# microsoft/aurora

Hardware: AMD Instinct MI355X
Metric: forecast-steps/sec (6h step) 0.25deg ERA5 721x1440x13 (higher is better)
Workload: dtype bf16; 1 GPU; AuroraPretrained(autocast=True) 1.3B, 0.25deg ERA5 721x1440, 13 levels, T=2, batch 1 per GPU, one forward step (BASELINE.json configs[1]); parallelism=1 GPU

## Files before the change

aurora_amd/csrc/model.h:

```cpp
#pragma once

#include <math.h>
#include <stdlib.h>
#include <string.h>

#include <algorithm>
#include <array>
#include <exception>
#include <map>
#include <memory>
#include <stdexcept>
#include <string>
#include <vector>

#include "band.h"
#include "common.h"

namespace aurora {

struct Fail {
  int code;
};
#define REQUIRE(cond, ...)               \
  do {                                   \
// ... 175 lines not shown
  std::vector<std::array<int, 2>> merge_pad;

  aurora_hip_band band{0, 1, nullptr, nullptr, nullptr};
  std::vector<std::vector<std::array<int, 2>>> rows;
  std::map<std::pair<int, int>, aurora::DevPlan> plans;
  void* stage_send = nullptr;
  void* stage_recv = nullptr;
  int64_t staging_bytes = 0, staging_need = 0;
  bool sharded() const { return band.world > 1; }
  int fuse_ln = 1;
  bool split_attention = false;
  bool qkv_planes = true;
  bool reassoc_out = true;
  bool compose_front = true;
  bool front_composed = false;
  bool score_weights = true;

  aurora::DevBuf abs_enc, dyn_planes, ctx_max;
  float guard_limit_min[4] = {INFINITY, INFINITY, INFINITY, INFINITY};
  int guard_launches[4] = {0, 0, 0, 0};
  void note_guard(const float* word, float limit) {
    const ptrdiff_t i = word - ctx_max.f();
    if (dry || word == nullptr || i < 0 || i >= 4) return;
    guard_limit_min[i] = std::min(guard_limit_min[i], limit);
    ++guard_launches[i];
  }
  aurora::DevBuf tickets;
  bool split_k = true;
  int abs_B = 0;
  struct Pinned { float* host = nullptr; size_t bytes = 0; hipEvent_t done = nullptr; };
// ... 125 lines not shown
    else linear(op.f32_mode(mode));
  }
  void linear_planes(const void* A, int64_t lda, const void* Wt, int64_t ldw, const float* bias, void* C, int64_t plane_stride,
                     int heads, int64_t M, int N, int K) {
    timed(m, stream, K_LINEAR_BF16, 2.0 * (double)M * N * K, [&] {
      return aurora_hip_linear_planes(A, lda, Wt, ldw, bias, C, plane_stride, heads, M, N, K, AURORA_BF16, stream);
    });
  }
  void layernorm(const void* y, int64_t ldy, const float* gain, const float* shift, const float* res, int64_t ldr,
                 int64_t res_mod, float* out_f32, int64_t ldo, void* out_t, int64_t ldt, int64_t M, int D, float eps,
                 int dtype) {
    timed(m, stream, K_LAYERNORM, 0.0, [&] {
      return aurora_hip_layernorm(y, ldy, gain, shift, res, ldr, res_mod, out_f32, ldo, out_t, ldt, M, D, eps, dtype, stream);
    });
  }
  void layernorm_split(const float* y, int64_t ldy, const float* gain, const float* shift, const void* res, int64_t ldr,
                       int64_t res_mod, int res_is_split, float* out_f32, int64_t ldo, void* out_split, int64_t ld_split,
                       int64_t M, int D, float eps) {
    timed(m, stream, K_LAYERNORM, 0.0, [&] {
      return aurora_hip_layernorm_split(y, ldy, gain, shift, res, ldr, res_mod, res_is_split, out_f32, ldo, out_split, ld_split, M, D,
                                        eps, stream);
    });
  }
  void perceiver_attention(const PerceiverCols& g, int head_dim, const float* q, int64_t q_stride, const float* kv, float* att,
                           const float* pair_word, float pair_limit, const float* skip_word, float skip_limit) {
    timed(m, stream, K_PERCEIVER_ATTENTION, 0.0, [&] {
      if (skip_word)
        return aurora_hip_perceiver_attention_unless(q, q_stride, kv, att, g.B, g.cols, g.kv_bstride, g.kv_lstride, g.Lq, g.Lk, g.heads,
                                                     head_dim, AURORA_F32, pair_word, pair_limit, skip_word, skip_limit, stream);
      return aurora_hip_perceiver_attention_ex(q, q_stride, kv, att, g.B, g.cols, g.kv_bstride, g.kv_lstride, g.Lq, g.Lk, g.heads,
// ... 81 lines not shown
```

aurora_amd/csrc/model.hip:

```cpp
#include "model.h"

namespace aurora {

hipEvent_t take_event(Model& m) {
  if (!m.event_pool.empty()) {
    hipEvent_t e = m.event_pool.back();
    m.event_pool.pop_back();
    return e;
  }
  hipEvent_t e;
  hip_ok(hipEventCreate(&e), "hipEventCreate");
  return e;
}

int bounded_mode() {
  static const int mode = getenv("AURORA_F32_GEMM") ? -1 : 2;
  return mode;
}

std::string level_to_str(double level) {
  const double value = round(level * 1000.0) / 1000.0;
  char buf[64];
  if (value == (double)(long long)value) snprintf(buf, sizeof buf, "%lld", (long long)value);
  else {
// ... 162 lines not shown
    build_channels(*m);
    m->ctx_max = DevBuf(16);
    const auto& tu = c->tuning;
    REQUIRE(tu.fuse_ln >= 0 && tu.fuse_ln <= 3, "create: tuning.fuse_ln = %d (0 default, 1 never, 2 by the fill rule, 3 always)", tu.fuse_ln);
    auto sw = [](int32_t v, bool dflt, const char* what) {
      REQUIRE(v >= 0 && v <= 2, "create: tuning.%s = %d (0 default, 1 off, 2 on)", what, v);
      return v == 0 ? dflt : v == 2;
    };
    m->fuse_ln = tu.fuse_ln == 0 ? 1 : tu.fuse_ln - 1;
    m->split_attention = sw(tu.band_split_attention, false, "band_split_attention");
    m->qkv_planes = sw(tu.qkv_planes, true, "qkv_planes");
    m->split_k = sw(tu.split_k, true, "split_k");
    m->reassoc_out = sw(tu.perceiver_reassoc, true, "perceiver_reassoc");
    m->score_weights = sw(tu.score_weights, true, "score_weights");
    m->compose_front = sw(tu.compose_front, true, "compose_front");
    m->tickets = DevBuf(SPLIT_TICKETS * sizeof(int32_t));
    hip_ok(hipMemset(m->tickets.p, 0, SPLIT_TICKETS * sizeof(int32_t)), "hipMemset");
    *out = m.release();
  })
}

extern "C" void aurora_hip_destroy(aurora_hip_model* m) { delete m; }

extern "C" int aurora_hip_set_band(aurora_hip_model* mp, const aurora_hip_band* band) {
  GUARDED({
    REQUIRE(mp != nullptr, "set_band: null model");
    Model& m = *mp;
    if (band == nullptr || band->world <= 1) {
      m.band = aurora_hip_band{0, 1, nullptr, nullptr, nullptr};
    } else {
// ... 168 lines not shown
```

aurora_amd/csrc/norm.hip:

```cpp
#include <stdlib.h>

#include "common.h"

namespace aurora {
namespace {

constexpr int ROWS_PER_BLOCK = 4;

template <int MAXC>
__device__ __forceinline__ void row_stats(const float (&v)[MAXC][8], int lane, int n_pieces, float inv_d, float eps,
                                          float& mean, float& rstd) {
  float s = 0.f;
#pragma unroll
  for (int i = 0; i < MAXC; ++i)
    if (lane + 64 * i < n_pieces) {
#pragma unroll
      for (int j = 0; j < 8; ++j) s += v[i][j];
    }
  mean = wave_sum(s) * inv_d;
  float q = 0.f;
#pragma unroll
  for (int i = 0; i < MAXC; ++i)
    if (lane + 64 * i < n_pieces) {
#pragma unroll
      for (int j = 0; j < 8; ++j) {
        const float d = v[i][j] - mean;
        q = fmaf(d, d, q);
      }
    }
  rstd = rsqrtf(wave_sum(q) * inv_d + eps);
}

struct LnArgs {
  const void* y; int64_t ldy; const float* gain; const float* shift;
  const float* res; int64_t ldr; int64_t res_mod;
  float* out_f32; int64_t ldo; void* out_t; int64_t ldt;
  int64_t M; int D; float eps;
  int split_t;
  int split_res;
};

template <typename T, int NC, bool PRE = false>
__global__ __launch_bounds__(256) void layernorm_f32_kernel(const LnArgs p) {
  const int lane = threadIdx.x & 63;
  const int64_t row = (int64_t)blockIdx.x * ROWS_PER_BLOCK + (threadIdx.x >> 6);
  if (row >= p.M) return;
  const int n_pieces = p.D >> 2;
  const T* yr = reinterpret_cast<const T*>(p.y) + row * p.ldy;
  const float* rr = nullptr;
  if (p.res) rr = p.res + (p.res_mod > 0 ? (int64_t)(((p.M | p.res_mod) >> 32) == 0 ? (uint32_t)row % (uint32_t)p.res_mod : row % p.res_mod) : row) * p.ldr;
  const bool res_plain = PRE && rr != nullptr && !p.split_res;
  float v[NC][4], r4[PRE ? NC : 1][4];
#pragma unroll
  for (int i = 0; i < NC; ++i)
    if (lane + 64 * i < n_pieces) {
      load4(yr + (lane + 64 * i) * 4, v[i]);
      if constexpr (PRE) {
        if (res_plain) load4(rr + (lane + 64 * i) * 4, r4[i]);
      }
    }
  float s = 0.f;
#pragma unroll
  for (int i = 0; i < NC; ++i)
    if (lane + 64 * i < n_pieces) s += (v[i][0] + v[i][1]) + (v[i][2] + v[i][3]);
  const float inv_d = 1.0f / p.D;
  const float mean = wave_sum(s) * inv_d;
  float q = 0.f;
#pragma unroll
  for (int i = 0; i < NC; ++i)
    if (lane + 64 * i < n_pieces) {
#pragma unroll
      for (int j = 0; j < 4; ++j) {
        const float d = v[i][j] - mean;
        q = fmaf(d, d, q);
      }
    }
  const float rstd = rsqrtf(wave_sum(q) * inv_d + p.eps);
#pragma unroll
  for (int i = 0; i < NC; ++i) {
    const int e = (lane + 64 * i) * 4;
    if (lane + 64 * i < n_pieces) {
      float gn[4], sh[4], o[4];
      if (p.gain) load4(p.gain + e, gn);
      if (p.shift) load4(p.shift + e, sh);
#pragma unroll
      for (int j = 0; j < 4; ++j) {
        float t = (v[i][j] - mean) * rstd;
        if (p.gain) t *= gn[j];
        if (p.shift) t += sh[j];
        o[j] = t;
      }
      if (rr && p.split_res) {
        const char* s = reinterpret_cast<const char*>(rr) + (e & ~31) * 4 + (e & 31) * 2;
        const u32x2 h = *reinterpret_cast<const u32x2*>(s);
        const u32x2 l = *reinterpret_cast<const u32x2*>(s + 64);
        auto half = [](uint32_t w, int hi) { return (float)__builtin_bit_cast(_Float16, (uint16_t)(hi ? w >> 16 : w & 0xffffu)); };
        const uint32_t hw[2] = {h.x, h.y}, lw[2] = {l.x, l.y};
#pragma unroll
        for (int j = 0; j < 4; ++j) o[j] += half(hw[j >> 1], j & 1) + half(lw[j >> 1], j & 1);
      } else if (rr) {
        if constexpr (PRE) {
#pragma unroll
          for (int j = 0; j < 4; ++j) o[j] += r4[i][j];
        } else {
          float r[4];
          load4(rr + e, r);
#pragma unroll
          for (int j = 0; j < 4; ++j) o[j] += r[j];
        }
      }
      if (p.out_f32) store4(p.out_f32 + row * p.ldo + e, o);
      if (p.out_t && p.split_t) {
        uint32_t h0, h1, l0, l1;
        split_pair_f16(o[0], o[1], h0, l0);
        split_pair_f16(o[2], o[3], h1, l1);
        const bool odd = (lane & 1) != 0;
        auto swap1 = [](uint32_t x) { return (uint32_t)__builtin_amdgcn_update_dpp(0, (int)x, 0xB1, 0xf, 0xf, true); };
        const uint32_t r0 = swap1(odd ? h0 : l0), r1 = swap1(odd ? h1 : l1);
        const int e8 = e & ~7;
        char* d = reinterpret_cast<char*>(p.out_t) + (row * p.ldt + (e8 & ~31)) * 4 + (e8 & 31) * 2 + (odd ? 64 : 0);
        *reinterpret_cast<u32x4*>(d) = odd ? u32x4{r0, r1, l0, l1} : u32x4{h0, h1, r0, r1};
      } else if (p.out_t) {
        store4(reinterpret_cast<T*>(p.out_t) + row * p.ldt + e, o);
      }
    }
  }
}

struct MergeArgs {
  const float* x; const float* w; const float* b; void* out;
  int B, C, H, W, D, H2, W2; float eps;
};

template <typename T, int MAXC>
__global__ __launch_bounds__(256) void merge_ln_kernel(const MergeArgs p) {
  const int lane = threadIdx.x & 63;
  const int64_t row = (int64_t)blockIdx.x * ROWS_PER_BLOCK + (threadIdx.x >> 6);
  const int64_t rows = (int64_t)p.B * p.C * p.H2 * p.W2;
  if (row >= rows) return;
// ... 77 lines not shown
}
}

using namespace aurora;

#define AURORA_DISPATCH_ROW(KERNEL, T, D, ...)                                                        \
  do {                                                                                                \
    if ((D) <= 512) hipLaunchKernelGGL((KERNEL<T, 1>), __VA_ARGS__);                                  \
    else if ((D) <= 1024) hipLaunchKernelGGL((KERNEL<T, 2>), __VA_ARGS__);                            \
    else if ((D) <= 2048) hipLaunchKernelGGL((KERNEL<T, 4>), __VA_ARGS__);                            \
    else hipLaunchKernelGGL((KERNEL<T, 8>), __VA_ARGS__);                                             \
  } while (0)

static int layernorm_impl(const void* y, int64_t ldy, const float* gain, const float* shift, const float* res, int64_t ldr,
                          int64_t res_mod, float* out_f32, int64_t ldo, void* out_t, int64_t ldt, int64_t M, int D,
                          float eps, int dtype, int split_t, int split_res, void* stream);

extern "C" int aurora_hip_layernorm(const void* y, int64_t ldy, const float* gain, const float* shift,
                                    const float* res, int64_t ldr, int64_t res_mod, float* out_f32,
                                    int64_t ldo, void* out_t, int64_t ldt, int64_t M, int D, float eps,
                                    int dtype, void* stream) {
  return layernorm_impl(y, ldy, gain, shift, res, ldr, res_mod, out_f32, ldo, out_t, ldt, M, D, eps, dtype, 0, 0, stream);
}

extern "C" int aurora_hip_layernorm_split(const float* y, int64_t ldy, const float* gain, const float* shift,
                                          const void* res, int64_t ldr, int64_t res_mod, int res_is_split, float* out_f32,
                                          int64_t ldo, void* out_split, int64_t ld_split, int64_t M, int D, float eps,
                                          void* stream) {
  AURORA_CHECK_ARG(D % 32 == 0, "layernorm_split: D=%d must be a multiple of 32", D);
  AURORA_CHECK_ARG(out_split == nullptr || (ld_split % 32 == 0 && ld_split >= D),
                   "layernorm_split: the pair-layout output stride must be a multiple of 32, >= D");
  AURORA_CHECK_ARG(!res_is_split || (res != nullptr && ldr % 32 == 0 && ldr >= D),
                   "layernorm_split: the pair-layout residual stride must be a multiple of 32, >= D");
  return layernorm_impl(y, ldy, gain, shift, static_cast<const float*>(res), ldr, res_mod, out_f32, ldo, out_split, ld_split,
                        M, D, eps, AURORA_F32, out_split ? 1 : 0, res_is_split ? 1 : 0, stream);
}

static int layernorm_impl(const void* y, int64_t ldy, const float* gain, const float* shift, const float* res, int64_t ldr,
                          int64_t res_mod, float* out_f32, int64_t ldo, void* out_t, int64_t ldt, int64_t M, int D,
                          float eps, int dtype, int split_t, int split_res, void* stream) {
  AURORA_CHECK_ARG(dtype == AURORA_F32 || dtype == AURORA_BF16, "layernorm: bad dtype");
  AURORA_CHECK_ARG(D % 8 == 0 && D > 0 && D <= 4096, "layernorm: D=%d must be a multiple of 8, <= 4096", D);
  const int es = dtype == AURORA_F32 ? 4 : 2;
  AURORA_CHECK_ARG((ldy * es) % 16 == 0 && (uintptr_t)y % 16 == 0, "layernorm: unaligned input rows");
  AURORA_CHECK_ARG((!res || ((ldr * 4) % 16 == 0 && (uintptr_t)res % 16 == 0)) &&
                       (!out_f32 || ((ldo * 4) % 16 == 0 && (uintptr_t)out_f32 % 16 == 0)) &&
                       (!out_t || ((ldt * es) % 16 == 0 && (uintptr_t)out_t % 16 == 0)),
                   "layernorm: unaligned residual/output rows");
  AURORA_CHECK_ARG(out_f32 || out_t, "layernorm: no output");
  if (M <= 0) return AURORA_OK;
  LnArgs p{y, ldy, gain, shift, res, ldr, res_mod, out_f32, ldo, out_t, ldt, M, D, eps, split_t, split_res};
  if (dtype == AURORA_F32) {
    const dim3 grid(row_blocks(M)), block(256);
    if (D <= 256) hipLaunchKernelGGL((layernorm_f32_kernel<float, 1>), grid, block, 0, as_stream(stream), p);
    else if (D <= 512) hipLaunchKernelGGL((layernorm_f32_kernel<float, 2>), grid, block, 0, as_stream(stream), p);
    else if (D <= 1024) hipLaunchKernelGGL((layernorm_f32_kernel<float, 4>), grid, block, 0, as_stream(stream), p);
    else if (D <= 2048) hipLaunchKernelGGL((layernorm_f32_kernel<float, 8>), grid, block, 0, as_stream(stream), p);
    else hipLaunchKernelGGL((layernorm_f32_kernel<float, 16>), grid, block, 0, as_stream(stream), p);
  } else {
    const dim3 grid(row_blocks(M)), block(256);
    const bool pre = res != nullptr && M <= (int64_t)40 * device_cus();
    if (pre) {
      if (D <= 256) hipLaunchKernelGGL((layernorm_f32_kernel<bf16_t, 1, true>), grid, block, 0, as_stream(stream), p);
      else if (D <= 512) hipLaunchKernelGGL((layernorm_f32_kernel<bf16_t, 2, true>), grid, block, 0, as_stream(stream), p);
      else if (D <= 1024) hipLaunchKernelGGL((layernorm_f32_kernel<bf16_t, 4, true>), grid, block, 0, as_stream(stream), p);
      else if (D <= 2048) hipLaunchKernelGGL((layernorm_f32_kernel<bf16_t, 8, true>), grid, block, 0, as_stream(stream), p);
// ... 41 lines not shown
```

aurora_amd/csrc/step.hip:

```cpp
#include <algorithm>

#include "model.h"
#include "resampler_space.h"

namespace aurora {

namespace {

struct CtxGuard { float* word; float a, c, limit_kv; bool pairs, scan; };
struct ComposedFront { const ComposedCtx* layers; int levels, groups; int64_t rows; float embed_l1, embed_bias_max; };

struct ResamplerCall {
  const Resampler* rs;
  const float* ctx;
  int64_t ctx_rows;
  int ctx_dim;
  const float *q0, *latents0;
  PerceiverCols g;
  float eps;
  bool out_pairs;
  const ComposedFront* front;
  CtxGuard guard;
};

// ... 445 lines not shown
    window_attention(s, blk, qkv, plane_stride, ao, (const int32_t*)pl.tok.p, pl.has_grp ? (const uint8_t*)pl.grp.p : nullptr,
                     pl.n_windows, pl.n_tok, Lq, Ls);
  return ao;
}

void block(Step& s, const Block& blk, const void* w_qkv, const void* w_proj, int stage, float* xf, void* xb, float* final_out,
           int64_t final_ld) {
  Model& m = s.m;
  Launcher& L = s.L;
  Arena& A = m.arena;
  const Res res = s.local_res(stage);
  const int64_t Ls = (int64_t)res.c * res.h * res.w, M = (int64_t)s.B * Ls;
  const int dim = blk.dim, bb = s.bb;
  const size_t es = s.es;
  const void* a_in = s.bf ? xb : (const void*)xf;
  const size_t mark = A.top;
  void* ao = s.sharded ? attention_band(s, blk, w_qkv, stage, a_in, Ls) : attention_whole(s, blk, w_qkv, stage, a_in, Ls);
  const int fuse_env = m.fuse_ln;
  const int64_t ln_tiles = (M + 127) / 128, cus = device_cus();
  const bool fills = (double)ln_tiles >= 0.85 * (double)(((ln_tiles + cus - 1) / cus) * cus);
  const bool fuse = s.bf && dim == 512 && (fuse_env == 2 || (fuse_env == 1 && fills));
  auto fused = [&](const void* a, const void* w, const float* bias, int K_, const float* gain, const float* shift, float* xo,
                   int64_t ldo, void* xbo) {
    timed(m, L.stream, K_LINEAR_LN, 2.0 * (double)M * dim * K_, [&] {
      return aurora_hip_linear_layernorm(a, K_, w, K_, bias, gain, shift, xf, dim, xo, ldo, xbo, dim, M, dim, K_, 1e-5f, L.stream);
    });
  };
  if (fuse) {
    fused(ao, w_proj, blk.proj_b, dim, blk.gain1, blk.shift1, xf, dim, xb);
  } else {
    void* y = A.take((size_t)M * dim * es);
    L.linear(LinearOp(ao, dim, w_proj, dim, blk.proj_b, y, dim, M, dim, dim, bb));
    L.layernorm(y, dim, blk.gain1, blk.shift1, xf, dim, 0, xf, dim, xb, dim, M, dim, 1e-5f, bb);
  }
  A.top = mark;
  void* hid = A.take((size_t)M * blk.hidden * es);
  L.linear(LinearOp(a_in, dim, blk.fc1_w, dim, blk.fc1_b, hid, blk.hidden, M, blk.hidden, dim, bb).activation(AURORA_ACT_GELU));
  float* xo = final_out ? final_out : xf;
  const int64_t ldo = final_out ? final_ld : dim;
  void* xbo = final_out ? nullptr : xb;
  if (fuse) {
    fused(hid, blk.fc2_w, blk.fc2_b, blk.hidden, blk.gain2, blk.shift2, xo, ldo, xbo);
  } else {
    void* y2 = A.take((size_t)M * dim * es);
    L.linear(LinearOp(hid, blk.hidden, blk.fc2_w, blk.hidden, blk.fc2_b, y2, dim, M, dim, blk.hidden, bb));
    L.layernorm(y2, dim, blk.gain2, blk.shift2, xf, dim, 0, xo, ldo, xbo, dim, M, dim, 1e-5f, bb);
  }
  A.top = mark;
}

void merge_stage(Step& s, int i, float*& xf, void*& xb) {
  Model& m = s.m;
  Arena& A = m.arena;
  const Res g = m.stage_res[i], r = s.local_res(i);
  REQUIRE(g.h > 1 && g.w > 1, "grid (%d, %d, %d) too small to merge", g.c, g.h, g.w);
  const int dim = m.stage_dim(i);
  const int H2 = (r.h + 1) / 2, W2 = (r.w + 1) / 2;
  REQUIRE(H2 == s.local_res(i + 1).h, "band rows of stages %d / %d do not nest", i, i + 1);
  const int64_t M2 = (int64_t)s.B * r.c * H2 * W2;
  float* nf = (float*)A.take((size_t)M2 * 2 * dim * 4);
  void* nb = s.bf ? A.take((size_t)M2 * 2 * dim * 2) : nullptr;
// ... 248 lines not shown
```

aurora_amd/engine/lib.py:

```python

from __future__ import annotations

import ctypes
import os
import threading
from collections import namedtuple
from ctypes import c_float, c_int, c_int32, c_int64, c_void_p
from pathlib import Path
from typing import Optional

import numpy as np
import torch

from aurora_amd.engine.tables import DeviceTables, _upload

F32, BF16, F64 = 0, 1, 2
ACT_NONE, ACT_GELU, ACT_SILU = 0, 1, 2

_LIB_PATH = Path(__file__).resolve().parents[1] / "_lib" / "libaurora_hip.so"


class PatchVar(ctypes.Structure):
    _fields_ = [
        ("src", c_void_p), ("stride_b", c_int64), ("stride_t", c_int64), ("stride_c", c_int64),
# ... 31 lines not shown
    "aurora_hip_linear_batched": (c_int, [c_void_p, c_int64, c_void_p, c_int64, c_void_p, c_void_p, c_int64, c_int64, c_int,
                                          c_int, c_int, c_int, c_int, c_void_p, c_float, c_int, c_int64, c_int64, c_int64,
                                          c_int64, c_void_p]),
    "aurora_hip_linear_plan": (c_int, [c_int64, c_int, c_int, c_int, c_int, c_int, c_int, c_int64, c_int64, c_int64, c_int64,
                                       c_int64, c_int64, c_int64, c_int, c_int, c_int64, c_int, c_int,
                                       ctypes.POINTER(c_int32)]),
    "aurora_hip_absmax": (c_int, [c_void_p, c_int64, c_void_p, c_void_p]),
    "aurora_hip_absmax_fold": (c_int, [c_void_p, c_int64, c_void_p, c_void_p]),
    "aurora_hip_zero_words": (c_int, [c_void_p, c_int, c_void_p]),
    "aurora_hip_linear_layernorm": (c_int, [c_void_p, c_int64, c_void_p, c_int64, c_void_p, c_void_p, c_void_p, c_void_p,
                                            c_int64, c_void_p, c_int64, c_void_p, c_int64, c_int64, c_int, c_int, c_float,
                                            c_void_p]),
    "aurora_hip_split_f16": (c_int, [c_void_p, c_int64, c_void_p, c_int64, c_int64, c_int, c_float, c_void_p]),
    "aurora_hip_layernorm_split": (c_int, [c_void_p, c_int64, c_void_p, c_void_p, c_void_p, c_int64, c_int64, c_int,
                                           c_void_p, c_int64, c_void_p, c_int64, c_int64, c_int, c_float, c_void_p]),
    "aurora_hip_linear": (c_int, [c_void_p, c_int64, c_void_p, c_int64, c_void_p, c_void_p, c_int64,
                                  c_void_p, c_int64, c_void_p, c_int64, c_int64, c_int, c_int, c_int,
                                  c_int, c_void_p]),
    "aurora_hip_window_attention": (c_int, [c_void_p, c_void_p, c_void_p, c_void_p, c_void_p, c_int,
                                            c_int64, c_int64, c_int, c_int, c_int, c_int, c_int, c_void_p]),
    "aurora_hip_window_attention_planes": (c_int, [c_void_p, c_int64, c_void_p, c_void_p, c_void_p, c_void_p, c_int,
                                                   c_int64, c_int64, c_int, c_int, c_int, c_int, c_int, c_void_p]),
    "aurora_hip_linear_planes": (c_int, [c_void_p, c_int64, c_void_p, c_int64, c_void_p, c_void_p, c_int64, c_int, c_int64,
                                         c_int, c_int, c_int, c_void_p]),
    "aurora_hip_gather_rows": (c_int, [c_void_p, c_int64, c_void_p, c_void_p, c_int64, c_int64, c_int64,
                                       c_void_p]),
    "aurora_hip_layernorm": (c_int, [c_void_p, c_int64, c_void_p, c_void_p, c_void_p, c_int64, c_int64,
                                     c_void_p, c_int64, c_void_p, c_int64, c_int64, c_int, c_float,
                                     c_int, c_void_p]),
    "aurora_hip_merge_ln": (c_int, [c_void_p, c_void_p, c_void_p, c_void_p, c_int, c_int, c_int, c_int,
# ... 429 lines not shown
    nbytes = M * D * (y.element_size() + (4 if res is not None else 0) + (4 if out_f32 is not None else 0)
                      + (y.element_size() if out_t is not None else 0))
    if split_t or split_res:
        assert y.dtype == torch.float32 and (out_t is not None) == split_t and (res is not None or not split_res)
        with _Timed("layernorm", float(nbytes)):
            _check(load().aurora_hip_layernorm_split(_ptr(y), ldy, _ptr(gain), _ptr(shift), _ptr(res), ldr, res_mod,
                                                     1 if split_res else 0, _ptr(out_f32), ldo, _ptr(out_t), ldt, M, D,
                                                     eps, _stream()))
        return
    with _Timed("layernorm", float(nbytes)):
        _check(load().aurora_hip_layernorm(_ptr(y), ldy, _ptr(gain), _ptr(shift), _ptr(res), ldr, res_mod,
                                           _ptr(out_f32), ldo, _ptr(out_t), ldt, M, D, eps,
                                           dtype_code(y.dtype), _stream()))


def merge_ln(x: torch.Tensor, ln_w: torch.Tensor, ln_b: torch.Tensor, out: torch.Tensor,
             B: int, C: int, H: int, W: int, D: int, eps: float = 1e-5) -> torch.Tensor:
    assert x.dtype == torch.float32 and x.is_contiguous() and x.numel() == B * C * H * W * D
    assert out.is_contiguous() and out.numel() == B * C * ((H + 1) // 2) * ((W + 1) // 2) * 4 * D
    with _Timed("merge_ln", 0.0):
        _check(load().aurora_hip_merge_ln(_ptr(x), _ptr(ln_w), _ptr(ln_b), _ptr(out), B, C, H, W, D, eps,
                                          dtype_code(out.dtype), _stream()))
    return out


def split_ln(y: torch.Tensor, ln_w: torch.Tensor, ln_b: torch.Tensor, out: torch.Tensor,
             B: int, C: int, H: int, W: int, Dq: int, crop_h: int, crop_w: int,
             eps: float = 1e-5) -> torch.Tensor:
    assert y.is_contiguous() and y.numel() == B * C * H * W * 4 * Dq and y.dtype == out.dtype
    assert out.is_contiguous() and out.numel() == B * C * (2 * H - crop_h) * (2 * W - crop_w) * Dq
# ... 809 lines not shown
                                   n_cols * (C * (1 + sum(k in addr for k in ("col_u", "col_v"))) +
                                             sum(k in addr for k in ("tcwv", "ivtu", "ivtv", "ivt"))))
    _launch(dev, "diagnostics", moved, "aurora_hip_diagnostics", at.get("u"), at.get("v"), at.get("vo"), at.get("div"), at.get("ws"), n_wind,
            _ptr(row_table), float(L), 1 if wrap else 0, at.get("q"), at.get("col_u"), at.get("col_v"), at.get("tcwv"), at.get("ivtu"),
            at.get("ivtv"), at.get("ivt"), n_cols, C, _ptr(level_w), n_lat, n_lon)


_PD = ctypes.POINTER(ctypes.c_double)
_PF = ctypes.POINTER(ctypes.c_float)
_PS = ctypes.POINTER(ctypes.c_char_p)


class HipTuning(ctypes.Structure):
    _fields_ = [("fuse_ln", c_int32), ("band_split_attention", c_int32), ("qkv_planes", c_int32), ("split_k", c_int32),
                ("perceiver_reassoc", c_int32), ("score_weights", c_int32), ("compose_front", c_int32),
                ("reserved", c_int32 * 1)]


def tuning_from_env() -> HipTuning:
    t = HipTuning()

    def value(var: str, allowed: tuple[int, ...]):
        raw = os.environ.get(var)
        if raw is None:
            return None
        try:
            v = int(raw.strip())
        except ValueError:
            v = None
        if v not in allowed:
            raise ValueError(f"{var}={raw!r}: expected one of {', '.join(map(str, allowed))}")
        return v

    v = value("AURORA_FUSE_LN", (0, 1, 2))
    if v is not None:
        t.fuse_ln = v + 1
    for field, var in (("band_split_attention", "AURORA_BAND_SPLIT_ATTENTION"), ("qkv_planes", "AURORA_QKV_PLANES"),
                       ("split_k", "AURORA_SPLIT_K"), ("perceiver_reassoc", "AURORA_PERCEIVER_REASSOC"),
                       ("score_weights", "AURORA_SCORE_WEIGHTS"), ("compose_front", "AURORA_COMPOSE_FRONT")):
        v = value(var, (0, 1))
        if v is not None:
            setattr(t, field, 2 if v else 1)
    return t


class HipConfig(ctypes.Structure):
    _fields_ = [("embed_dim", c_int32), ("patch_size", c_int32), ("latent_levels", c_int32), ("num_heads", c_int32),
                ("n_stages", c_int32), ("encoder_depths", c_int32 * 4), ("encoder_heads", c_int32 * 4),
                ("decoder_depths", c_int32 * 4), ("decoder_heads", c_int32 * 4), ("window", c_int32 * 3),
                ("enc_depth", c_int32), ("dec_depth", c_int32), ("perceiver_ln_eps", c_float),
                ("max_history", c_int32), ("timestep_hours", ctypes.c_double), ("stabilise_level_agg", c_int32),
                ("use_lora", c_int32), ("lora_steps", c_int32), ("lora_mode", c_int32), ("autocast", c_int32),
                ("n_surf", c_int32), ("n_static", c_int32), ("n_atmos", c_int32),
                ("surf_vars", _PS), ("static_vars", _PS), ("atmos_vars", _PS),
# ... 93 lines not shown
```

include/aurora_hip.h:

```cpp
#ifndef AURORA_HIP_H
#define AURORA_HIP_H

#include <stddef.h>
#include <stdint.h>

#ifdef __cplusplus
extern "C" {
#endif

#define AURORA_F32 0
#define AURORA_BF16 1
#define AURORA_F64 2

#define AURORA_OK 0
#define AURORA_E_ARG (-1)
#define AURORA_E_LAUNCH (-2)

#define AURORA_ACT_NONE 0
#define AURORA_ACT_GELU 1
#define AURORA_ACT_SILU 2

const char* aurora_hip_last_error(void);
int aurora_hip_version(void);

// ... 59 lines not shown
                                       int B, int64_t L, int64_t L_out, int D, int heads, int n_windows,
                                       int win_tokens, int dtype, void* stream);

int aurora_hip_layernorm(const void* y, int64_t ldy, const float* gain, const float* shift,
                         const float* res, int64_t ldr, int64_t res_mod,
                         float* out_f32, int64_t ldo, void* out_t, int64_t ldt,
                         int64_t M, int D, float eps, int dtype, void* stream);
int aurora_hip_linear_layernorm(const void* A, int64_t lda, const void* W, int64_t ldw, const float* bias,
                                const float* gain, const float* shift,
                                const float* x_in, int64_t ldx, float* x_out, int64_t ldo,
                                void* x_bf16, int64_t ldb, int64_t M, int N, int K, float eps, void* stream);

int aurora_hip_layernorm_split(const float* y, int64_t ldy, const float* gain, const float* shift,
                               const void* res, int64_t ldr, int64_t res_mod, int res_is_split,
                               float* out_f32, int64_t ldo, void* out_split, int64_t ld_split,
                               int64_t M, int D, float eps, void* stream);

int aurora_hip_merge_ln(const float* x, const float* ln_w, const float* ln_b, void* out,
                        int B, int C, int H, int W, int D, float eps, int dtype, void* stream);

int aurora_hip_split_ln(const void* y, const float* ln_w, const float* ln_b, void* out,
                        int B, int C, int H, int W, int Dq, int crop_h, int crop_w, float eps,
                        int dtype, void* stream);

typedef struct aurora_patch_var {
  const float* src;
  int64_t stride_b;
  int64_t stride_t;
  int64_t stride_c;
  int64_t stride_h;
// ... 96 lines not shown
  int32_t n_modulation_heads;    const char* const* modulation_heads;
  const int32_t* difference_history;
  int32_t n_positive_surf;       const char* const* positive_surf_vars;
  int32_t n_positive_atmos;      const char* const* positive_atmos_vars;
  int32_t n_surf_inputs;         const char* const* surf_inputs;
  int32_t n_density;             const char* const* density_channel_surf_vars;
  int32_t n_angle;               const char* const* angle_surf_vars;
  struct aurora_hip_tuning {
    int32_t fuse_ln;
    int32_t band_split_attention;
    int32_t qkv_planes;
    int32_t split_k;
    int32_t perceiver_reassoc;
    int32_t score_weights;
    int32_t compose_front;
    int32_t reserved[1];
  } tuning;
} aurora_hip_config;

typedef struct aurora_hip_grid {
  int32_t n_lat, n_lon;
  const double* lat;
  const double* lon;
  int32_t n_levels;
  const double* levels;
  int32_t levels_float32;
  const double* surf_loc;
  const double* surf_scale;
  const double* static_loc;
  const double* static_scale;
  const double* atmos_loc;
// ... 182 lines not shown
```

Before: 7.990 forecast-steps/s.

## Carry first post-norm as stats and recompute it in the second layernorm

In each Swin block's post-norm residual path (bf16, non-fused case), the first layernorm no longer writes the updated fp32 residual. It writes only the bf16 activation plus per-row mean/rstd. The second layernorm recomputes x1 from the saved projection output, the stats and the original residual, then applies the second norm, so the fp32 write and re-read of the intermediate residual are skipped. In exchange it adds a bf16 buffer read and extra gain/shift loads, and it forces an unfused add order that may change rounding slightly.

```diff
diff --git a/aurora_amd/csrc/model.h b/aurora_amd/csrc/model.h
--- a/aurora_amd/csrc/model.h
+++ b/aurora_amd/csrc/model.h
@@ -213,6 +213,7 @@
   bool reassoc_out = true;
   bool compose_front = true;
   bool front_composed = false;
+  bool ln_carry = true;
   bool score_weights = true;
 
   aurora::DevBuf abs_enc, dyn_planes, ctx_max;
@@ -368,6 +369,20 @@
       return aurora_hip_layernorm(y, ldy, gain, shift, res, ldr, res_mod, out_f32, ldo, out_t, ldt, M, D, eps, dtype, stream);
     });
   }
+  void layernorm_stats(const void* y, int64_t ldy, const float* gain, const float* shift, const float* res, int64_t ldr, void* out_t,
+                       int64_t ldt, float* stats, int64_t M, int D, float eps, int dtype) {
+    timed(m, stream, K_LAYERNORM, 0.0, [&] {
+      return aurora_hip_layernorm_stats(y, ldy, gain, shift, res, ldr, out_t, ldt, stats, M, D, eps, dtype, stream);
+    });
+  }
+  void layernorm_carry(const void* y2, const void* y1, const float* stats1, const Block& blk, const float* x0, float* out_f32,
+                       int64_t ldo, void* out_bf16, int64_t M, float eps) {
+    const int D = blk.dim;
+    timed(m, stream, K_LAYERNORM, 0.0, [&] {
+      return aurora_hip_layernorm_carry(y2, D, y1, D, stats1, blk.gain1, blk.shift1, blk.gain2, blk.shift2, x0, D, out_f32, ldo,
+                                        out_bf16, D, M, D, eps, stream);
+    });
+  }
   void layernorm_split(const float* y, int64_t ldy, const float* gain, const float* shift, const void* res, int64_t ldr,
                        int64_t res_mod, int res_is_split, float* out_f32, int64_t ldo, void* out_split, int64_t ld_split,
                        int64_t M, int D, float eps) {
diff --git a/aurora_amd/csrc/model.hip b/aurora_amd/csrc/model.hip
--- a/aurora_amd/csrc/model.hip
+++ b/aurora_amd/csrc/model.hip
@@ -200,6 +200,7 @@
     m->reassoc_out = sw(tu.perceiver_reassoc, true, "perceiver_reassoc");
     m->score_weights = sw(tu.score_weights, true, "score_weights");
     m->compose_front = sw(tu.compose_front, true, "compose_front");
+    m->ln_carry = sw(tu.ln_carry, true, "ln_carry");
     m->tickets = DevBuf(SPLIT_TICKETS * sizeof(int32_t));
     hip_ok(hipMemset(m->tickets.p, 0, SPLIT_TICKETS * sizeof(int32_t)), "hipMemset");
     *out = m.release();
diff --git a/aurora_amd/csrc/norm.hip b/aurora_amd/csrc/norm.hip
--- a/aurora_amd/csrc/norm.hip
+++ b/aurora_amd/csrc/norm.hip
@@ -29,6 +29,36 @@
       }
     }
   rstd = rsqrtf(wave_sum(q) * inv_d + eps);
+}
+
+__device__ __forceinline__ float ln_update(float y, float mean, float rstd, float gain, float shift, float res) {
+#pragma clang fp contract(off)
+  float t = (y - mean) * rstd;
+  t = t * gain;
+  t = t + shift;
+  return t + res;
+}
+
+template <int NC>
+__device__ __forceinline__ void row_stats4(const float (&v)[NC][4], int lane, int n_pieces, int D, float eps, float& mean,
+                                           float& rstd) {
+  float s = 0.f;
+#pragma unroll
+  for (int i = 0; i < NC; ++i)
+    if (lane + 64 * i < n_pieces) s += (v[i][0] + v[i][1]) + (v[i][2] + v[i][3]);
+  const float inv_d = 1.0f / D;
+  mean = wave_sum(s) * inv_d;
+  float q = 0.f;
+#pragma unroll
+  for (int i = 0; i < NC; ++i)
+    if (lane + 64 * i < n_pieces) {
+#pragma unroll
+      for (int j = 0; j < 4; ++j) {
+        const float d = v[i][j] - mean;
+        q = fmaf(d, d, q);
+      }
+    }
+  rstd = rsqrtf(fmaf(wave_sum(q), inv_d, eps));
 }
 
 struct LnArgs {
@@ -38,6 +68,7 @@
   int64_t M; int D; float eps;
   int split_t;
   int split_res;
+  float* stats;
 };
 
 template <typename T, int NC, bool PRE = false>
@@ -59,37 +90,16 @@
         if (res_plain) load4(rr + (lane + 64 * i) * 4, r4[i]);
       }
     }
-  float s = 0.f;
-#pragma unroll
-  for (int i = 0; i < NC; ++i)
-    if (lane + 64 * i < n_pieces) s += (v[i][0] + v[i][1]) + (v[i][2] + v[i][3]);
-  const float inv_d = 1.0f / p.D;
-  const float mean = wave_sum(s) * inv_d;
-  float q = 0.f;
-#pragma unroll
-  for (int i = 0; i < NC; ++i)
-    if (lane + 64 * i < n_pieces) {
-#pragma unroll
-      for (int j = 0; j < 4; ++j) {
-        const float d = v[i][j] - mean;
-        q = fmaf(d, d, q);
-      }
-    }
-  const float rstd = rsqrtf(wave_sum(q) * inv_d + p.eps);
+  float mean, rstd;
+  row_stats4<NC>(v, lane, n_pieces, p.D, p.eps, mean, rstd);
+  if (p.stats && lane == 0) *reinterpret_cast<f32x2_hw*>(p.stats + 2 * row) = f32x2_hw{mean, rstd};
 #pragma unroll
   for (int i = 0; i < NC; ++i) {
     const int e = (lane + 64 * i) * 4;
     if (lane + 64 * i < n_pieces) {
-      float gn[4], sh[4], o[4];
+      float gn[4], sh[4], r[4], o[4];
       if (p.gain) load4(p.gain + e, gn);
       if (p.shift) load4(p.shift + e, sh);
-#pragma unroll
-      for (int j = 0; j < 4; ++j) {
-        float t = (v[i][j] - mean) * rstd;
-        if (p.gain) t *= gn[j];
-        if (p.shift) t += sh[j];
-        o[j] = t;
-      }
       if (rr && p.split_res) {
         const char* s = reinterpret_cast<const char*>(rr) + (e & ~31) * 4 + (e & 31) * 2;
         const u32x2 h = *reinterpret_cast<const u32x2*>(s);
@@ -97,18 +107,18 @@
         auto half = [](uint32_t w, int hi) { return (float)__builtin_bit_cast(_Float16, (uint16_t)(hi ? w >> 16 : w & 0xffffu)); };
         const uint32_t hw[2] = {h.x, h.y}, lw[2] = {l.x, l.y};
 #pragma unroll
-        for (int j = 0; j < 4; ++j) o[j] += half(hw[j >> 1], j & 1) + half(lw[j >> 1], j & 1);
+        for (int j = 0; j < 4; ++j) r[j] = half(hw[j >> 1], j & 1) + half(lw[j >> 1], j & 1);
       } else if (rr) {
         if constexpr (PRE) {
 #pragma unroll
-          for (int j = 0; j < 4; ++j) o[j] += r4[i][j];
+          for (int j = 0; j < 4; ++j) r[j] = r4[i][j];
         } else {
-          float r[4];
           load4(rr + e, r);
-#pragma unroll
-          for (int j = 0; j < 4; ++j) o[j] += r[j];
         }
       }
+#pragma unroll
+      for (int j = 0; j < 4; ++j)
+        o[j] = ln_update(v[i][j], mean, rstd, p.gain ? gn[j] : 1.0f, p.shift ? sh[j] : -0.0f, rr ? r[j] : -0.0f);
       if (p.out_f32) store4(p.out_f32 + row * p.ldo + e, o);
       if (p.out_t && p.split_t) {
         uint32_t h0, h1, l0, l1;
@@ -123,6 +133,66 @@
       } else if (p.out_t) {
         store4(reinterpret_cast<T*>(p.out_t) + row * p.ldt + e, o);
       }
+    }
+  }
+}
+
+struct CarryArgs {
+  const bf16_t* y2; int64_t ldy2; const bf16_t* y1; int64_t ldy1; const float* stats1;
+  const float *gain1, *shift1, *gain2, *shift2;
+  const float* x0; int64_t ldx;
+  float* out_f32; int64_t ldo; bf16_t* out_t; int64_t ldt;
+  int64_t M; int D; float eps;
+};
+
+template <int NC, bool PRE>
+__global__ __launch_bounds__(256) void layernorm_carry_kernel(const CarryArgs p) {
+  const int lane = threadIdx.x & 63;
+  const int64_t row = (int64_t)blockIdx.x * ROWS_PER_BLOCK + (threadIdx.x >> 6);
+  if (row >= p.M) return;
+  const int n_pieces = p.D >> 2;
+  const bf16_t* y2r = p.y2 + row * p.ldy2;
+  const bf16_t* y1r = p.y1 + row * p.ldy1;
+  const float* xr = p.x0 + row * p.ldx;
+  float v[NC][4], r4[PRE ? NC : 1][4];
+  u32x2 u2[PRE ? NC : 1];
+#pragma unroll
+  for (int i = 0; i < NC; ++i)
+    if (lane + 64 * i < n_pieces) {
+      load4(y2r + (lane + 64 * i) * 4, v[i]);
+      if constexpr (PRE) {
+        u2[i] = *reinterpret_cast<const u32x2*>(y1r + (lane + 64 * i) * 4);
+        load4(xr + (lane + 64 * i) * 4, r4[i]);
+      }
+    }
+  const f32x2_hw st1 = *reinterpret_cast<const f32x2_hw*>(p.stats1 + 2 * row);
+  float mean2, rstd2;
+  row_stats4<NC>(v, lane, n_pieces, p.D, p.eps, mean2, rstd2);
+#pragma unroll
+  for (int i = 0; i < NC; ++i) {
+    const int e = (lane + 64 * i) * 4;
+    if (lane + 64 * i < n_pieces) {
+      float g1[4], s1[4], g2[4], s2[4], a[4], r[4], o[4];
+      if constexpr (PRE) {
+        a[0] = __uint_as_float(u2[i].x << 16); a[1] = __uint_as_float(u2[i].x & 0xffff0000u);
+        a[2] = __uint_as_float(u2[i].y << 16); a[3] = __uint_as_float(u2[i].y & 0xffff0000u);
+#pragma unroll
+        for (int j = 0; j < 4; ++j) r[j] = r4[i][j];
+      } else {
+        load4(y1r + e, a);
+        load4(xr + e, r);
+      }
+      load4(p.gain1 + e, g1);
+      load4(p.shift1 + e, s1);
+      load4(p.gain2 + e, g2);
+      load4(p.shift2 + e, s2);
+#pragma unroll
+      for (int j = 0; j < 4; ++j) {
+        const float x1 = ln_update(a[j], st1.x, st1.y, g1[j], s1[j], r[j]);
+        o[j] = ln_update(v[i][j], mean2, rstd2, g2[j], s2[j], x1);
+      }
+      if (p.out_f32) store4(p.out_f32 + row * p.ldo + e, o);
+      if (p.out_t) store4(p.out_t + row * p.ldt + e, o);
     }
   }
 }
@@ -230,13 +300,13 @@
 
 static int layernorm_impl(const void* y, int64_t ldy, const float* gain, const float* shift, const float* res, int64_t ldr,
                           int64_t res_mod, float* out_f32, int64_t ldo, void* out_t, int64_t ldt, int64_t M, int D,
-                          float eps, int dtype, int split_t, int split_res, void* stream);
+                          float eps, int dtype, int split_t, int split_res, float* stats, void* stream);
 
 extern "C" int aurora_hip_layernorm(const void* y, int64_t ldy, const float* gain, const float* shift,
                                     const float* res, int64_t ldr, int64_t res_mod, float* out_f32,
                                     int64_t ldo, void* out_t, int64_t ldt, int64_t M, int D, float eps,
                                     int dtype, void* stream) {
-  return layernorm_impl(y, ldy, gain, shift, res, ldr, res_mod, out_f32, ldo, out_t, ldt, M, D, eps, dtype, 0, 0, stream);
+  return layernorm_impl(y, ldy, gain, shift, res, ldr, res_mod, out_f32, ldo, out_t, ldt, M, D, eps, dtype, 0, 0, nullptr, stream);
 }
 
 extern "C" int aurora_hip_layernorm_split(const float* y, int64_t ldy, const float* gain, const float* shift,
@@ -249,12 +319,52 @@
   AURORA_CHECK_ARG(!res_is_split || (res != nullptr && ldr % 32 == 0 && ldr >= D),
                    "layernorm_split: the pair-layout residual stride must be a multiple of 32, >= D");
   return layernorm_impl(y, ldy, gain, shift, static_cast<const float*>(res), ldr, res_mod, out_f32, ldo, out_split, ld_split,
-                        M, D, eps, AURORA_F32, out_split ? 1 : 0, res_is_split ? 1 : 0, stream);
+                        M, D, eps, AURORA_F32, out_split ? 1 : 0, res_is_split ? 1 : 0, nullptr, stream);
+}
+
+extern "C" int aurora_hip_layernorm_stats(const void* y, int64_t ldy, const float* gain, const float* shift, const float* res,
+                                          int64_t ldr, void* out_t, int64_t ldt, float* stats, int64_t M, int D, float eps,
+                                          int dtype, void* stream) {
+  AURORA_CHECK_ARG(out_t != nullptr && stats != nullptr, "layernorm_stats: no output");
+  return layernorm_impl(y, ldy, gain, shift, res, ldr, 0, nullptr, 0, out_t, ldt, M, D, eps, dtype, 0, 0, stats, stream);
+}
+
+extern "C" int aurora_hip_layernorm_carry(const void* y2, int64_t ldy2, const void* y1, int64_t ldy1, const float* stats1,
+                                          const float* gain1, const float* shift1, const float* gain2, const float* shift2,
+                                          const float* x0, int64_t ldx, float* out_f32, int64_t ldo, void* out_bf16,
+                                          int64_t ldt, int64_t M, int D, float eps, void* stream) {
+  AURORA_CHECK_ARG(D % 8 == 0 && D > 0 && D <= 4096, "layernorm_carry: D=%d must be a multiple of 8, <= 4096", D);
+  AURORA_CHECK_ARG(y2 && y1 && stats1 && gain1 && shift1 && gain2 && shift2 && x0, "layernorm_carry: null operand");
+  AURORA_CHECK_ARG(out_f32 || out_bf16, "layernorm_carry: no output");
+  auto rows16 = [](const void* ptr, int64_t ld, int es) { return !ptr || ((ld * es) % 16 == 0 && (uintptr_t)ptr % 16 == 0); };
+  AURORA_CHECK_ARG(rows16(y2, ldy2, 2) && rows16(y1, ldy1, 2) && rows16(x0, ldx, 4) && rows16(out_f32, ldo, 4) && rows16(out_bf16, ldt, 2) &&
+                       (uintptr_t)stats1 % 8 == 0 && (uintptr_t)gain1 % 16 == 0 && (uintptr_t)shift1 % 16 == 0 &&
+                       (uintptr_t)gain2 % 16 == 0 && (uintptr_t)shift2 % 16 == 0,
+                   "layernorm_carry: unaligned rows");
+  AURORA_CHECK_ARG(ldy2 >= D && ldy1 >= D && ldx >= D && (!out_f32 || ldo >= D) && (!out_bf16 || ldt >= D),
+                   "layernorm_carry: a row stride is smaller than D=%d", D);
+  if (M <= 0) return AURORA_OK;
+  CarryArgs p{static_cast<const bf16_t*>(y2), ldy2, static_cast<const bf16_t*>(y1), ldy1, stats1, gain1, shift1, gain2, shift2,
+              x0, ldx, out_f32, ldo, static_cast<bf16_t*>(out_bf16), ldt, M, D, eps};
+  const dim3 grid(row_blocks(M)), block(256);
+  const bool pre = M <= (int64_t)40 * device_cus();
+#define AURORA_CARRY(NC)                                                                                               \
+  do {                                                                                                                 \
+    if (pre) hipLaunchKernelGGL((layernorm_carry_kernel<NC, true>), grid, block, 0, as_stream(stream), p);            \
+    else hipLaunchKernelGGL((layernorm_carry_kernel<NC, false>), grid, block, 0, as_stream(stream), p);                \
+  } while (0)
+  if (D <= 256) AURORA_CARRY(1);
+  else if (D <= 512) AURORA_CARRY(2);
+  else if (D <= 1024) AURORA_CARRY(4);
+  else if (D <= 2048) AURORA_CARRY(8);
+  else hipLaunchKernelGGL((layernorm_carry_kernel<16, false>), grid, block, 0, as_stream(stream), p);
+#undef AURORA_CARRY
+  return check_launch("layernorm_carry");
 }
 
 static int layernorm_impl(const void* y, int64_t ldy, const float* gain, const float* shift, const float* res, int64_t ldr,
                           int64_t res_mod, float* out_f32, int64_t ldo, void* out_t, int64_t ldt, int64_t M, int D,
-                          float eps, int dtype, int split_t, int split_res, void* stream) {
+                          float eps, int dtype, int split_t, int split_res, float* stats, void* stream) {
   AURORA_CHECK_ARG(dtype == AURORA_F32 || dtype == AURORA_BF16, "layernorm: bad dtype");
   AURORA_CHECK_ARG(D % 8 == 0 && D > 0 && D <= 4096, "layernorm: D=%d must be a multiple of 8, <= 4096", D);
   const int es = dtype == AURORA_F32 ? 4 : 2;
@@ -264,8 +374,9 @@
                        (!out_t || ((ldt * es) % 16 == 0 && (uintptr_t)out_t % 16 == 0)),
                    "layernorm: unaligned residual/output rows");
   AURORA_CHECK_ARG(out_f32 || out_t, "layernorm: no output");
+  AURORA_CHECK_ARG(!stats || (uintptr_t)stats % 8 == 0, "layernorm: unaligned statistics");
   if (M <= 0) return AURORA_OK;
-  LnArgs p{y, ldy, gain, shift, res, ldr, res_mod, out_f32, ldo, out_t, ldt, M, D, eps, split_t, split_res};
+  LnArgs p{y, ldy, gain, shift, res, ldr, res_mod, out_f32, ldo, out_t, ldt, M, D, eps, split_t, split_res, stats};
   if (dtype == AURORA_F32) {
     const dim3 grid(row_blocks(M)), block(256);
     if (D <= 256) hipLaunchKernelGGL((layernorm_f32_kernel<float, 1>), grid, block, 0, as_stream(stream), p);
diff --git a/aurora_amd/csrc/step.hip b/aurora_amd/csrc/step.hip
--- a/aurora_amd/csrc/step.hip
+++ b/aurora_amd/csrc/step.hip
@@ -483,12 +483,16 @@
   const int dim = blk.dim, bb = s.bb;
   const size_t es = s.es;
   const void* a_in = s.bf ? xb : (const void*)xf;
-  const size_t mark = A.top;
-  void* ao = s.sharded ? attention_band(s, blk, w_qkv, stage, a_in, Ls) : attention_whole(s, blk, w_qkv, stage, a_in, Ls);
   const int fuse_env = m.fuse_ln;
   const int64_t ln_tiles = (M + 127) / 128, cus = device_cus();
   const bool fills = (double)ln_tiles >= 0.85 * (double)(((ln_tiles + cus - 1) / cus) * cus);
   const bool fuse = s.bf && dim == 512 && (fuse_env == 2 || (fuse_env == 1 && fills));
+  const bool carry = s.bf && !fuse && m.ln_carry;
+  const size_t mark = A.top;
+  void* y1 = carry ? A.take((size_t)M * dim * es) : nullptr;
+  float* stats1 = carry ? (float*)A.take((size_t)M * 2 * sizeof(float)) : nullptr;
+  const size_t kept = A.top;
+  void* ao = s.sharded ? attention_band(s, blk, w_qkv, stage, a_in, Ls) : attention_whole(s, blk, w_qkv, stage, a_in, Ls);
   auto fused = [&](const void* a, const void* w, const float* bias, int K_, const float* gain, const float* shift, float* xo,
                    int64_t ldo, void* xbo) {
     timed(m, L.stream, K_LINEAR_LN, 2.0 * (double)M * dim * K_, [&] {
@@ -498,11 +502,12 @@
   if (fuse) {
     fused(ao, w_proj, blk.proj_b, dim, blk.gain1, blk.shift1, xf, dim, xb);
   } else {
-    void* y = A.take((size_t)M * dim * es);
+    void* y = carry ? y1 : A.take((size_t)M * dim * es);
     L.linear(LinearOp(ao, dim, w_proj, dim, blk.proj_b, y, dim, M, dim, dim, bb));
-    L.layernorm(y, dim, blk.gain1, blk.shift1, xf, dim, 0, xf, dim, xb, dim, M, dim, 1e-5f, bb);
-  }
-  A.top = mark;
+    if (carry) L.layernorm_stats(y, dim, blk.gain1, blk.shift1, xf, dim, xb, dim, stats1, M, dim, 1e-5f, bb);
+    else L.layernorm(y, dim, blk.gain1, blk.shift1, xf, dim, 0, xf, dim, xb, dim, M, dim, 1e-5f, bb);
+  }
+  A.top = kept;
   void* hid = A.take((size_t)M * blk.hidden * es);
   L.linear(LinearOp(a_in, dim, blk.fc1_w, dim, blk.fc1_b, hid, blk.hidden, M, blk.hidden, dim, bb).activation(AURORA_ACT_GELU));
   float* xo = final_out ? final_out : xf;
@@ -513,7 +518,8 @@
   } else {
     void* y2 = A.take((size_t)M * dim * es);
     L.linear(LinearOp(hid, blk.hidden, blk.fc2_w, blk.hidden, blk.fc2_b, y2, dim, M, dim, blk.hidden, bb));
-    L.layernorm(y2, dim, blk.gain2, blk.shift2, xf, dim, 0, xo, ldo, xbo, dim, M, dim, 1e-5f, bb);
+    if (carry) L.layernorm_carry(y2, y1, stats1, blk, xf, xo, ldo, xbo, M, 1e-5f);
+    else L.layernorm(y2, dim, blk.gain2, blk.shift2, xf, dim, 0, xo, ldo, xbo, dim, M, dim, 1e-5f, bb);
   }
   A.top = mark;
 }
diff --git a/aurora_amd/engine/lib.py b/aurora_amd/engine/lib.py
--- a/aurora_amd/engine/lib.py
+++ b/aurora_amd/engine/lib.py
@@ -69,6 +69,11 @@
     "aurora_hip_split_f16": (c_int, [c_void_p, c_int64, c_void_p, c_int64, c_int64, c_int, c_float, c_void_p]),
     "aurora_hip_layernorm_split": (c_int, [c_void_p, c_int64, c_void_p, c_void_p, c_void_p, c_int64, c_int64, c_int,
                                            c_void_p, c_int64, c_void_p, c_int64, c_int64, c_int, c_float, c_void_p]),
+    "aurora_hip_layernorm_stats": (c_int, [c_void_p, c_int64, c_void_p, c_void_p, c_void_p, c_int64, c_void_p, c_int64,
+                                           c_void_p, c_int64, c_int, c_float, c_int, c_void_p]),
+    "aurora_hip_layernorm_carry": (c_int, [c_void_p, c_int64, c_void_p, c_int64, c_void_p, c_void_p, c_void_p, c_void_p,
+                                           c_void_p, c_void_p, c_int64, c_void_p, c_int64, c_void_p, c_int64, c_int64, c_int,
+                                           c_float, c_void_p]),
     "aurora_hip_linear": (c_int, [c_void_p, c_int64, c_void_p, c_int64, c_void_p, c_void_p, c_int64,
                                   c_void_p, c_int64, c_void_p, c_int64, c_int64, c_int, c_int, c_int,
                                   c_int, c_void_p]),
@@ -528,6 +533,32 @@
                                            dtype_code(y.dtype), _stream()))
 
 
+def layernorm_stats(y: torch.Tensor, gain: torch.Tensor, shift: torch.Tensor, res: torch.Tensor, out_t: torch.Tensor,
+                    stats: torch.Tensor, eps: float = 1e-5) -> None:
+    (ldy, D), M = _rows(y), y.shape[0]
+    assert res.dtype == torch.float32 and out_t.dtype == y.dtype and out_t.shape[0] == M == res.shape[0]
+    assert stats.dtype == torch.float32 and stats.is_contiguous() and tuple(stats.shape) == (M, 2)
+    with _Timed("layernorm", float(M * D * (2 * y.element_size() + 4) + M * 8)):
+        _check(load().aurora_hip_layernorm_stats(_ptr(y), ldy, _ptr(gain), _ptr(shift), _ptr(res), _rows(res)[0], _ptr(out_t),
+                                                 _rows(out_t)[0], _ptr(stats), M, D, eps, dtype_code(y.dtype), _stream()))
+
+
+def layernorm_carry(y2: torch.Tensor, y1: torch.Tensor, stats1: torch.Tensor, gain1: torch.Tensor, shift1: torch.Tensor,
+                    gain2: torch.Tensor, shift2: torch.Tensor, x0: torch.Tensor, *, out_f32: Optional[torch.Tensor] = None,
+                    out_t: Optional[torch.Tensor] = None, eps: float = 1e-5) -> None:
+    (ldy2, D), M = _rows(y2), y2.shape[0]
+    assert y2.dtype == y1.dtype == torch.bfloat16 and x0.dtype == stats1.dtype == torch.float32 and y1.shape[0] == M
+    assert out_f32 is None or out_f32.dtype == torch.float32
+    assert out_t is None or out_t.dtype == torch.bfloat16
+    ldo = _rows(out_f32)[0] if out_f32 is not None else 0
+    ldt = _rows(out_t)[0] if out_t is not None else 0
+    nbytes = M * D * (2 + 2 + 4 + (4 if out_f32 is not None else 0) + (2 if out_t is not None else 0)) + M * 8
+    with _Timed("layernorm", float(nbytes)):
+        _check(load().aurora_hip_layernorm_carry(_ptr(y2), ldy2, _ptr(y1), _rows(y1)[0], _ptr(stats1), _ptr(gain1), _ptr(shift1),
+                                                 _ptr(gain2), _ptr(shift2), _ptr(x0), _rows(x0)[0], _ptr(out_f32), ldo,
+                                                 _ptr(out_t), ldt, M, D, eps, _stream()))
+
+
 def merge_ln(x: torch.Tensor, ln_w: torch.Tensor, ln_b: torch.Tensor, out: torch.Tensor,
              B: int, C: int, H: int, W: int, D: int, eps: float = 1e-5) -> torch.Tensor:
     assert x.dtype == torch.float32 and x.is_contiguous() and x.numel() == B * C * H * W * D
@@ -1367,7 +1398,7 @@
 class HipTuning(ctypes.Structure):
     _fields_ = [("fuse_ln", c_int32), ("band_split_attention", c_int32), ("qkv_planes", c_int32), ("split_k", c_int32),
                 ("perceiver_reassoc", c_int32), ("score_weights", c_int32), ("compose_front", c_int32),
-                ("reserved", c_int32 * 1)]
+                ("ln_carry", c_int32)]
 
 
 def tuning_from_env() -> HipTuning:
@@ -1390,7 +1421,8 @@
         t.fuse_ln = v + 1
     for field, var in (("band_split_attention", "AURORA_BAND_SPLIT_ATTENTION"), ("qkv_planes", "AURORA_QKV_PLANES"),
                        ("split_k", "AURORA_SPLIT_K"), ("perceiver_reassoc", "AURORA_PERCEIVER_REASSOC"),
-                       ("score_weights", "AURORA_SCORE_WEIGHTS"), ("compose_front", "AURORA_COMPOSE_FRONT")):
+                       ("score_weights", "AURORA_SCORE_WEIGHTS"), ("compose_front", "AURORA_COMPOSE_FRONT"),
+                       ("ln_carry", "AURORA_LN_CARRY")):
         v = value(var, (0, 1))
         if v is not None:
             setattr(t, field, 2 if v else 1)
diff --git a/include/aurora_hip.h b/include/aurora_hip.h
--- a/include/aurora_hip.h
+++ b/include/aurora_hip.h
@@ -97,6 +97,14 @@
 int aurora_hip_layernorm_split(const float* y, int64_t ldy, const float* gain, const float* shift,
                                const void* res, int64_t ldr, int64_t res_mod, int res_is_split,
                                float* out_f32, int64_t ldo, void* out_split, int64_t ld_split,
+                               int64_t M, int D, float eps, void* stream);
+
+int aurora_hip_layernorm_stats(const void* y, int64_t ldy, const float* gain, const float* shift,
+                               const float* res, int64_t ldr, void* out_t, int64_t ldt, float* stats,
+                               int64_t M, int D, float eps, int dtype, void* stream);
+int aurora_hip_layernorm_carry(const void* y2, int64_t ldy2, const void* y1, int64_t ldy1, const float* stats1,
+                               const float* gain1, const float* shift1, const float* gain2, const float* shift2,
+                               const float* x0, int64_t ldx, float* out_f32, int64_t ldo, void* out_bf16, int64_t ldt,
                                int64_t M, int D, float eps, void* stream);
 
 int aurora_hip_merge_ln(const float* x, const float* ln_w, const float* ln_b, void* out,
@@ -223,7 +231,7 @@
     int32_t perceiver_reassoc;
     int32_t score_weights;
     int32_t compose_front;
-    int32_t reserved[1];
+    int32_t ln_carry;
   } tuning;
 } aurora_hip_config;
 
```

Result: no change. 8.021 forecast-steps/s, median of 6 (+0.4%).
